# andrrizzi/tfep

Hardware: AMD Instinct MI355X
Metric: samples/s (fwd+log|detJ|) MAF+RQ-spline, 3N=3000, batch 64k (higher is better)
Workload: dtype f32

## Files before the change

include/tfep_hip.h:

```cpp
#ifndef TFEP_HIP_H
#define TFEP_HIP_H

#include <stdint.h>

#ifdef __cplusplus
extern "C" {
#endif

#define TFEP_HIP_ABI_VERSION 8

typedef enum tfep_status {
    TFEP_OK = 0,
    TFEP_ERR_INVALID_ARGUMENT = -1,
    TFEP_ERR_UNSUPPORTED = -2,
    TFEP_ERR_LAUNCH = -3
} tfep_status;

int tfep_hip_abi_version(void);
const char* tfep_last_error(void);

typedef struct tfep_param_layout {
    int64_t ld;
    int64_t stride_p;
    int64_t stride_f;
// ... 103 lines not shown

int tfep_quaternion_product(const float* x, int64_t ldx, const float* params, int64_t ldp, int inverse, float* y,
                            int64_t ldy, float* log_det_J, int accumulate, int B, int D, void* stream);

int tfep_periodic_embedding(const float* x, int64_t ldx, const int32_t* periodic_indices, int n_periodic,
                            const int32_t* nonperiodic_indices, int n_nonperiodic,
                            float lower, float upper, float* out, int64_t ldo, int B, void* stream);

int tfep_gather_columns(const float* src, int64_t lds, const int32_t* idx, int n_idx,
                        float* dst, int64_t ldd, int B, void* stream);
int tfep_scatter_columns(const float* src, int64_t lds, const int32_t* idx, int n_idx,
                         float* dst, int64_t ldd, int B, void* stream);


typedef enum tfep_fused_kind {
    TFEP_FUSED_AFFINE = 0,
    TFEP_FUSED_SPLINE = 1,
    TFEP_FUSED_SOS = 3
} tfep_fused_kind;

int tfep_fused_tile_features(void);
int tfep_fused_supported(int kind, const tfep_spline_desc* desc);
int tfep_fused_tile_columns(int kind, const tfep_spline_desc* desc);

int tfep_fused_output_transformer_forward(const float* h, int64_t ldh, const float* w, int64_t ldw,
                                          const float* bias_packed, const int32_t* k_ranges,
                                          const int32_t* tile_order,
                                          int kind, const tfep_spline_desc* desc,
                                          const float* x, int64_t ldx, float* y, int64_t ldy,
                                          const int32_t* feat_index, const int32_t* feat_tr,
                                          int n_feature_slots, double* ldj_partial,
                                          float* log_det_J, int accumulate,
                                          int B, int n_rows_w, int k_padded, void* stream);

int tfep_split_tile_k(void);
int tfep_split_rows(const float* src, int64_t ld_src, int64_t rows, int64_t cols, void* dst, int64_t ld_dst,
                    int64_t cols_padded, float* inv_scale, int per_tensor, void* stream);

int tfep_abs_reduce(const float* src, int64_t ld_src, int64_t rows, int64_t cols, int mode, float* out, void* stream);

int tfep_range_flag(const float* src, int64_t ld_src, int64_t rows, int64_t cols, int bits, int32_t* count, void* stream);
int tfep_column_absmax(const float* src, int64_t ld_src, int64_t rows, int64_t cols, float* out, void* stream);

int tfep_split_columns_scaled(const float* src, int64_t ld_src, int64_t rows, int64_t col0, int64_t cols, void* dst,
                              int64_t ld_dst, const float* inv_scale, void* stream);

int tfep_masked_weight_prepare_split(const float* weight_v, const float* weight_g, const float* mask, int out_features,
                                     int in_features, const int32_t* row_of_out, const int32_t* in_of_col, const int32_t* col_cut,
                                     void* w_split_out, int64_t ldw, int k_padded, float* inv_scale, void* stream);
int tfep_masked_weight_prepare_split_both(const float* weight_v, const float* weight_g, int out_features, int in_features,
                                          const int32_t* row_of_out, const int32_t* in_of_col, const int32_t* col_cut,
                                          void* w_split_out, int64_t ldw, float* w32_out, int64_t ldw32, int k_padded,
                                          float* inv_scale, void* stream);

int tfep_fused_output_transformer_forward_split(const void* h_split, int64_t ldh, const float* h_inv_scale,
                                                const void* w_split, int64_t ldw, const float* w_inv_scale,
                                                const float* bias_packed, const int32_t* k_ranges,
                                                const int32_t* tile_order, int kind, const tfep_spline_desc* desc,
                                                const float* x, int64_t ldx, float* y, int64_t ldy,
                                                const int32_t* feat_index, const int32_t* feat_tr, int n_feature_slots,
                                                double* ldj_partial, float* log_det_J, int accumulate, int B,
                                                int n_rows_w, int k_padded, void* stream);

int tfep_fused_saving_supported(const tfep_spline_desc* desc);
int tfep_fused_output_transformer_forward_split_saving(const void* h_split, int64_t ldh, const float* h_inv_scale,
                                                       const void* w_split, int64_t ldw, const float* w_inv_scale,
                                                       const float* bias_packed, const int32_t* k_ranges,
                                                       const int32_t* tile_order, const tfep_spline_desc* desc,
                                                       const float* x, int64_t ldx, float* y, int64_t ldy,
                                                       const int32_t* feat_index, const int32_t* feat_tr, int n_feature_slots,
                                                       double* ldj_partial, float* log_det_J, int accumulate, int B,
                                                       int n_rows_w, int k_padded, int w_feature_major, float* theta_out,
                                                       int64_t ld_theta, void* stream);

int tfep_diag_split_mfma_peak(float* scratch, int blocks, int iters, void* stream);
int tfep_diag_split_cycles(unsigned long long* out);

typedef struct tfep_inverse_block_desc {
    int32_t B, n_layers, n_steps, kind;
    float* x; int64_t ldx;
    float* xpad; int64_t ldxpad;
    const float* y; int64_t ldy;
    float* h[4]; int64_t ldh[4];
    const float* z[4]; int64_t ldz[4];
    const float* zout; int64_t ldzout;
    int32_t z_slabs[4]; int64_t z_slab_stride[4];
    int32_t zout_slabs; int64_t zout_slab_stride;
    float* log_det_J;
    const float* w[4]; int64_t ldw[4];
    const float* wout; int64_t ldwout;
    const int32_t* steps;
    const int32_t* feat_cols;
    const int32_t* feat_sel;
    const int32_t* feat_in;
    const int32_t* feat_periodic;
    const int32_t* in_cols;
    float emb_lower, emb_upper;
    int32_t cache_col0[4], cache_n_old[4];
    int32_t cache_len, max_feats;
    const tfep_spline_desc* spline;
    int32_t moebius_dim, moebius_unit_sphere;
    float moebius_max_radius;
    int32_t rows_per_wave;
    int32_t n_spline_groups;
    int32_t waves_per_workgroup;
    int32_t paired;
// ... 359 lines not shown
```

tfep_amd/_lib.py:

```python
import ctypes
import os
from ctypes import POINTER, Structure, c_char_p, c_double, c_float, c_int, c_int32, c_int64, c_void_p

import torch

_HERE = os.path.dirname(os.path.abspath(__file__))
LIB_PATH = os.environ.get('TFEP_HIP_LIB') or os.path.join(_HERE, 'lib', 'libtfep_hip.so')
ABI_VERSION = 8

_lib = None


class ParamLayout(Structure):
    _fields_ = [('ld', c_int64), ('stride_p', c_int64), ('stride_f', c_int64)]


class GemmDesc(Structure):
    _fields_ = [('x', c_void_p), ('ldx', c_int64), ('w', c_void_p), ('ldw', c_int64), ('bias', c_void_p),
                ('k_ranges', c_void_p), ('tile_order', c_void_p), ('col_map', c_void_p),
                ('y', c_void_p), ('ldy', c_int64),
                ('B', c_int32), ('N', c_int32), ('n_rows_w', c_int32), ('k_padded', c_int32),
                ('act', c_int32), ('accumulate', c_int32),
                ('elu_grad_of', c_void_p), ('ld_elu_grad_of', c_int64), ('tile_live', c_void_p),
                ('pre_add', c_void_p), ('ld_pre_add', c_int64), ('tile_n', c_int32),
# ... 39 lines not shown
                ('learn_lower_bound', c_int32), ('learn_upper_bound', c_int32),
                ('min_bin_size', c_float), ('min_slope', c_float)]


class SplineDescF64(Structure):
    _fields_ = [('x0', c_void_p), ('xf', c_void_p), ('y0', c_void_p), ('yf', c_void_p),
                ('n_bins', c_int32), ('circular', c_int32), ('identity_boundary_slopes', c_int32),
                ('learn_lower_bound', c_int32), ('learn_upper_bound', c_int32),
                ('min_bin_size', c_double), ('min_slope', c_double)]


class InverseChainF64Desc(Structure):
    _fields_ = [('B', c_int32), ('n_linears', c_int32), ('n_steps', c_int32), ('n_members', c_int32),
                ('y', c_void_p), ('ldy', c_int64), ('x', c_void_p), ('ldx', c_int64), ('log_det_J', c_void_p),
                ('a', c_void_p * 5), ('lda', c_int64 * 5), ('w', c_void_p * 5), ('ldw', c_int64 * 5), ('bias', c_void_p * 5),
                ('zout', c_void_p), ('ldzout', c_int64), ('zout_row0', c_int32), ('par_cols', c_int32), ('max_feats', c_int32),
                ('k0', c_int32 * 5), ('n_old', c_int32 * 5), ('n_cols', c_int32 * 5), ('lds_col0', c_int32 * 5),
                ('has_panel', c_int32 * 5), ('steps', c_void_p), ('feats', c_void_p), ('member_kind', c_int32 * 4),
                ('spline', SplineDescF64 * 4), ('emb_lower', c_double), ('emb_scale', c_double)]


class EgnnLayerParams(Structure):
    _fields_ = [('F', c_int32), ('G', c_int32)] + [(k, c_void_p) for k in (
        'dist_means', 'dist_log_gammas', 'msg0_w', 'msg0_b', 'msg2_w', 'msg2_b', 'att_w', 'att_b', 'ux0_w', 'ux0_b',
        'ux2_w', 'uh0_w', 'uh0_b', 'uh2_w', 'uh2_b')]


class EgnnEdgeArgs(Structure):
    _fields_ = [('B', c_int32), ('n_nodes', c_int32), ('nt', c_int32), ('split', c_int32), ('r_cutoff', c_float),
                ('speed_factor', c_float),
                ('packed', c_void_p), ('pos', c_void_p), ('dpos', c_void_p), ('P', c_void_p), ('Q', c_void_p),
                ('pq_bstride', c_int64), ('dP', c_void_p), ('dQ', c_void_p), ('pos_out', c_void_p), ('dpos_out', c_void_p),
                ('nm', c_void_p), ('dnm', c_void_p)]


class EgnnNodeArgs(Structure):
    _fields_ = [('B', c_int32), ('n_nodes', c_int32), ('nt', c_int32), ('packed', c_void_p), ('packed_next', c_void_p),
                ('h', c_void_p), ('h_bstride', c_int64), ('dh', c_void_p), ('nm', c_void_p), ('dnm', c_void_p),
                ('h_out', c_void_p), ('dh_out', c_void_p), ('P_out', c_void_p), ('Q_out', c_void_p),
                ('dP_out', c_void_p), ('dQ_out', c_void_p)]


class EgnnEdgeBwdArgs(Structure):
    _fields_ = [('B', c_int32), ('n_nodes', c_int32), ('nt', c_int32), ('split', c_int32), ('src_owned', c_int32),
                ('r_cutoff', c_float), ('speed_factor', c_float), ('packed', c_void_p), ('pos', c_void_p),
                ('P', c_void_p), ('Q', c_void_p), ('pq_bstride', c_int64), ('g_pos_out', c_void_p), ('g_nm', c_void_p),
                ('g_lane', c_void_p), ('g_pos', c_void_p)]


class EgnnNodeBwdArgs(Structure):
    _fields_ = [('B', c_int32), ('n_nodes', c_int32), ('nt', c_int32), ('packed', c_void_p), ('packed_next', c_void_p),
                ('h', c_void_p), ('h_bstride', c_int64), ('nm', c_void_p), ('g_h_next', c_void_p), ('g_P', c_void_p),
                ('g_Q', c_void_p), ('g_h', c_void_p), ('g_nm', c_void_p)]


_P = c_void_p
_SIGNATURES = {
    'tfep_hip_abi_version': (c_int, []),
    'tfep_last_error': (c_char_p, []),
    'tfep_masked_weight_prepare': (c_int, [_P, _P, _P, c_int, c_int, _P, _P, _P, c_int, _P, c_int, c_int64, _P]),
    'tfep_masked_weight_prepare_prefix': (c_int, [_P, _P, c_int, c_int, _P, _P, _P, _P, c_int, c_int64, _P]),
    'tfep_mask_k_ranges': (c_int, [_P, c_int, c_int, _P, _P, c_int, c_int, c_int, c_int, _P, _P]),
    'tfep_masked_linear_forward': (c_int, [_P, c_int64, _P, c_int64, _P, _P, _P, _P, _P, c_int64,
                                           c_int, c_int, c_int, c_int, c_int, c_int, _P]),
    'tfep_masked_linear_narrow_tile_n': (c_int, []),
    'tfep_masked_linear_tile_n': (c_int, []),
    'tfep_split_wide_tile_n': (c_int, []),
    'tfep_split_half_wide_tile_n': (c_int, []),
    'tfep_masked_linear_tile_k': (c_int, []),
    'tfep_masked_linear_tile_m': (c_int, []),
    'tfep_affine_forward': (c_int, [_P, c_int64, _P, ParamLayout, _P, c_int64, _P, c_int, c_int, c_int, _P]),
    'tfep_affine_inverse': (c_int, [_P, c_int64, _P, ParamLayout, _P, c_int64, _P, c_int, c_int, c_int, _P]),
    'tfep_sos_forward': (c_int, [_P, c_int64, _P, ParamLayout, c_int, _P, c_int64, _P, c_int, c_int, c_int, _P]),
    'tfep_sos_backward': (c_int, [_P, c_int64, _P, ParamLayout, c_int, _P, c_int64, _P, ParamLayout, _P, c_int64,
                                  c_int, c_int, _P]),
    'tfep_volume_preserving_shift': (c_int, [_P, c_int64, _P, c_int64, _P, c_float, c_float, c_int,
                                             _P, c_int64, c_int, c_int, _P]),
    'tfep_spline_n_parameters_per_feature': (c_int, [POINTER(SplineDesc)]),
    'tfep_spline_forward': (c_int, [_P, c_int64, _P, ParamLayout, POINTER(SplineDesc), _P, c_int64,
                                    _P, c_int, c_int, c_int, _P]),
    'tfep_spline_inverse': (c_int, [_P, c_int64, _P, ParamLayout, POINTER(SplineDesc), _P, c_int64,
                                    _P, c_int, c_int, c_int, _P]),
    'tfep_moebius_forward': (c_int, [_P, c_int64, _P, c_int64, c_int, c_float, c_int, c_int,
                                     _P, c_int64, _P, c_int, c_int, c_int, _P]),
    'tfep_symmetrized_moebius': (c_int, [_P, c_int64, _P, c_int64, c_int, c_double, c_int, _P, c_int64, _P, c_int, c_int,
                                         c_int, _P]),
    'tfep_symmetrized_moebius_backward': (c_int, [_P, c_int64, _P, c_int64, c_int, c_double, c_int, _P, c_int64, _P, _P,
                                                  c_int64, _P, c_int64, c_int, c_int, _P]),
    'tfep_symmetrized_moebius_f64': (c_int, [_P, c_int64, _P, c_int64, c_int, c_double, c_int, _P, c_int64, _P, c_int, c_int,
                                             c_int, _P]),
    'tfep_symmetrized_moebius_backward_f64': (c_int, [_P, c_int64, _P, c_int64, c_int, c_double, c_int, _P, c_int64, _P, _P,
                                                      c_int64, _P, c_int64, c_int, c_int, _P]),
    'tfep_quaternion_product': (c_int, [_P, c_int64, _P, c_int64, c_int, _P, c_int64, _P, c_int, c_int, c_int, _P]),
    'tfep_quaternion_product_backward': (c_int, [_P, c_int64, _P, c_int64, c_int, _P, c_int64, _P, c_int64, _P, c_int64,
                                                 c_int, c_int, _P]),
    'tfep_quaternion_product_f64': (c_int, [_P, c_int64, _P, c_int64, c_int, _P, c_int64, _P, c_int, c_int, c_int, _P]),
    'tfep_quaternion_product_backward_f64': (c_int, [_P, c_int64, _P, c_int64, c_int, _P, c_int64, _P, c_int64, _P, c_int64,
                                                     c_int, c_int, _P]),
    'tfep_moebius_forward_split_out': (c_int, [_P, c_int64, _P, c_int64, c_float, _P, c_int64, _P, c_int, _P, c_int64, _P,
                                               c_int, c_int, _P]),
    'tfep_periodic_embedding': (c_int, [_P, c_int64, _P, c_int, _P, c_int, c_float, c_float,
                                        _P, c_int64, c_int, _P]),
    'tfep_gather_columns': (c_int, [_P, c_int64, _P, c_int, _P, c_int64, c_int, _P]),
    'tfep_scatter_columns': (c_int, [_P, c_int64, _P, c_int, _P, c_int64, c_int, _P]),
    'tfep_fused_tile_features': (c_int, []),
    'tfep_fused_supported': (c_int, [c_int, POINTER(SplineDesc)]),
    'tfep_fused_tile_columns': (c_int, [c_int, POINTER(SplineDesc)]),
    'tfep_fused_output_transformer_forward': (c_int, [_P, c_int64, _P, c_int64, _P, _P, _P, c_int,
                                                      POINTER(SplineDesc), _P, c_int64, _P, c_int64,
                                                      _P, _P, c_int, _P, _P, c_int,
                                                      c_int, c_int, c_int, _P]),
    'tfep_split_tile_k': (c_int, []),
    'tfep_masked_weight_prepare_split': (c_int, [_P, _P, _P, c_int, c_int, _P, _P, _P, _P, c_int64, c_int, _P, _P]),
    'tfep_masked_weight_prepare_split_both': (c_int, [_P, _P, c_int, c_int, _P, _P, _P, _P, c_int64, _P, c_int64, c_int, _P, _P]),
    'tfep_split_rows': (c_int, [_P, c_int64, c_int64, c_int64, _P, c_int64, c_int64, _P, c_int, _P]),
    'tfep_abs_reduce': (c_int, [_P, c_int64, c_int64, c_int64, c_int, _P, _P]),
    'tfep_range_flag': (c_int, [_P, c_int64, c_int64, c_int64, c_int, _P, _P]),
    'tfep_column_absmax': (c_int, [_P, c_int64, c_int64, c_int64, _P, _P]),
    'tfep_split_columns_scaled': (c_int, [_P, c_int64, c_int64, c_int64, c_int64, _P, c_int64, _P, _P]),
    'tfep_fused_output_transformer_forward_split': (c_int, [_P, c_int64, _P, _P, c_int64, _P, _P, _P, _P, c_int,
                                                            POINTER(SplineDesc), _P, c_int64, _P, c_int64,
                                                            _P, _P, c_int, _P, _P, c_int,
                                                            c_int, c_int, c_int, _P]),
    'tfep_fused_saving_supported': (c_int, [POINTER(SplineDesc)]),
    'tfep_fused_output_transformer_forward_split_saving': (c_int, [_P, c_int64, _P, _P, c_int64, _P, _P, _P, _P,
                                                                   POINTER(SplineDesc), _P, c_int64, _P, c_int64,
                                                                   _P, _P, c_int, _P, _P, c_int,
                                                                   c_int, c_int, c_int, c_int, _P, c_int64, _P]),
    'tfep_diag_split_mfma_peak': (c_int, [_P, c_int, c_int, _P]),
    'tfep_diag_split_cycles': (c_int, [_P]),
    'tfep_inverse_block_step_ints': (c_int, []),
    'tfep_inverse_block_record_ints': (c_int, []),
    'tfep_inverse_block_lds_bytes': (c_int64, [c_int, c_int, c_int]),
    'tfep_inverse_block_lds_bytes_rows': (c_int64, [c_int, c_int, c_int, c_int]),
    'tfep_inverse_block_lds_bytes_paired': (c_int64, [c_int, c_int, c_int]),
    'tfep_inverse_block': (c_int, [POINTER(InverseBlockDesc), _P]),
    'tfep_diag_inverse_cycles': (c_int, [_P]),
    'tfep_maf_layer_tile_n': (c_int, []),
    'tfep_maf_layer_forward_split': (c_int, [POINTER(MafLayerDesc), _P]),
    'tfep_diag_maf_layer_cycles': (c_int, [_P]),
    'tfep_diag_mfma_peak': (c_int, [_P, c_int, c_int, _P]),
    'tfep_masked_linear_gemm': (c_int, [POINTER(GemmDesc), _P]),
    'tfep_transpose': (c_int, [_P, c_int64, c_int, c_int, _P, c_int64, _P]),
    'tfep_transpose_split': (c_int, [_P, c_int64, c_int, c_int, _P, c_int64, c_int, c_int, _P, _P, _P]),
    'tfep_transpose_split_rows': (c_int, [_P, c_int64, c_int, c_int, _P, c_int64, _P]),
    'tfep_column_sums_absmax': (c_int, [_P, c_int64, c_int, c_int, _P, c_int, _P, _P]),
    'tfep_column_sums': (c_int, [_P, c_int64, c_int, c_int, _P, c_int, _P]),
    'tfep_add_inplace': (c_int, [_P, c_int64, _P, c_int64, c_int, c_int, _P]),
    'tfep_affine_backward': (c_int, [_P, c_int64, _P, ParamLayout, _P, c_int64, _P, _P, ParamLayout, _P, c_int64,
                                     c_int, c_int, _P]),
    'tfep_spline_backward': (c_int, [_P, c_int64, _P, ParamLayout, POINTER(SplineDesc), _P, c_int64, _P, _P,
                                     ParamLayout, _P, c_int64, c_int, c_int, _P]),
    'tfep_moebius_backward': (c_int, [_P, c_int64, _P, c_int64, c_int, c_float, c_int, c_int, _P, c_int64, _P,
                                      _P, c_int64, _P, c_int64, c_int, c_int, _P]),
    'tfep_copy_2d': (c_int, [_P, c_int64, _P, c_int64, c_int, c_int, _P]),
    'tfep_weight_norm_backward': (c_int, [_P, c_int64, _P, _P, _P, c_int, c_int, _P, _P, _P, _P, _P]),
    'tfep_weight_norm_backward_prefix': (c_int, [_P, c_int64, _P, _P, c_int, c_int, _P, _P, _P, _P, _P, _P]),
    'tfep_periodic_embedding_backward': (c_int, [_P, c_int64, _P, c_int, _P, c_int, c_float, c_float, _P, c_int64,
                                                 _P, c_int64, c_int, _P]),
    'tfep_tfep_reduce': (c_int, [_P, _P, _P, _P, _P, c_float, c_int, c_int, _P, _P, _P]),
    'tfep_tfep_reduce_workspace_doubles': (c_int, [c_int]),
    'tfep_bootstrap_fep': (c_int, [_P, _P, _P, _P, c_int64, c_int64, c_int64, c_float, _P, _P]),
    'tfep_egnn_tile': (c_int, [c_int, c_int]),
    'tfep_egnn_packed_floats': (c_int64, [c_int]),
    'tfep_egnn_pack_layer': (c_int, [POINTER(EgnnLayerParams), c_int, _P, _P]),
    'tfep_egnn_embed': (c_int, [_P, c_int, c_int, c_float, _P, _P, c_int, _P, _P, POINTER(EgnnLayerParams), c_int,
# ... 138 lines not shown
```

tfep_amd/build.py:

```python
import fcntl
import os
import subprocess
import sys

HERE = os.path.dirname(os.path.abspath(__file__))
CSRC = os.path.join(HERE, 'csrc')
LIB_DIR = os.path.join(HERE, 'lib')
LIB_PATH = os.path.join(LIB_DIR, 'libtfep_hip.so')
SOURCES = ['transformers.hip', 'masked_linear.hip', 'split_gemm.hip', 'split_gemm_layouts.hip', 'inverse_block.hip',
           'reduce.hip', 'backward.hip', 'egnn.hip', 'maf_layer.hip', 'masked_linear_f64.hip',
           'spline_f64.hip', 'inverse_block_f64.hip', 'flipembed.hip']
EXTRA_FLAGS = {'egnn.hip': ['-fno-slp-vectorize']}


def _hipcc():
    for cand in (os.environ.get('HIPCC'), '/opt/rocm/bin/hipcc', 'hipcc'):
        if cand and (os.path.isabs(cand) and os.path.exists(cand) or not os.path.isabs(cand)):
            return cand
    raise RuntimeError('hipcc not found')


def _headers():
    deps = [os.path.join(CSRC, f) for f in os.listdir(CSRC) if f.endswith('.h')]
    deps.append(os.path.join(os.path.dirname(HERE), 'include', 'tfep_hip.h'))
    return deps


def needs_build():
    if not os.path.exists(LIB_PATH):
        return True
    t = os.path.getmtime(LIB_PATH)
    deps = [os.path.join(CSRC, f) for f in SOURCES] + _headers()
    return any(os.path.getmtime(d) > t for d in deps)


def build_probe(out_path, extra_flags, verbose=True):
    import tempfile
    tmp = tempfile.mkdtemp(prefix='tfep_probe_')
    objs, procs = [], []
    for src in SOURCES:
        obj = os.path.join(tmp, src.replace('.hip', '.o'))
        objs.append(obj)
        cmd = [_hipcc(), '-O3', '-std=c++17', '--offload-arch=gfx950', '-fPIC', '-fno-gpu-rdc', '-Wno-unused-result',
               *EXTRA_FLAGS.get(src, []), *extra_flags, '-c', os.path.join(CSRC, src), '-o', obj]
        if verbose:
            print(' '.join(cmd), flush=True)
        procs.append((src, subprocess.Popen(cmd)))
    for src, p in procs:
        if p.wait() != 0:
            raise RuntimeError(f'hipcc failed on {src}')
    subprocess.check_call([_hipcc(), '--offload-arch=gfx950', '-shared', '-fPIC', '-o', out_path] + objs)
    return out_path


def build(force=False, verbose=True):
    if not force and not needs_build():
        return LIB_PATH
    os.makedirs(LIB_DIR, exist_ok=True)
    with open(os.path.join(LIB_DIR, '.build.lock'), 'w') as lock:
        fcntl.flock(lock, fcntl.LOCK_EX)
        try:
            if not force and not needs_build():
                return LIB_PATH
            return _build_locked(force, verbose)
# ... 46 lines not shown
```

tfep_amd/nn/conditioners/made.py:

```python
from typing import Literal, Optional, Sequence, Union

import os

import numpy as np

import torch

from ... import ops
from ...utils.misc import ensure_tensor_sequence
from .. import masked
from .conditioner import Conditioner



def _round_robin(x, length, err_msg=None):
    n_rounds, n_rem = divmod(length, len(x))
    if n_rounds == 0:
        if err_msg is None:
            err_msg = f'Length {length} is smaller than the array (len={len(x)}).'
        raise ValueError(err_msg)
    out = x.repeat(n_rounds)
    if n_rem != 0:
        out = torch.cat([out, x[:n_rem]])
    return out
# ... 414 lines not shown
            old = plan.get('packed_fingerprint')
            stale = old is None or not torch.equal(old, fingerprint)
        plan['packed_checked'] = fingerprint
        if stale:
            for k in [k for k in plan if isinstance(k, tuple) and k[0] in ('packed', 'packed_split')]:
                del plan[k]
            plan['packed_versions'] = versions
        plan['packed_fingerprint'] = fingerprint
        return True

    def begin_call(self):
        self.__dict__['_fp_memo'] = None

    def _param_fingerprint(self):
        parts = []
        for lin in self._linears():
            for t in lin.parameters():
                flat = t.detach().reshape(-1)
                parts.append(flat[::1021].sum(dtype=torch.float64))
                parts.append(flat[:64].sum(dtype=torch.float64))
        return torch.stack(parts) if parts else torch.zeros(0)

    def _mask_prefix_cuts(self, plan, li, lin):
        if os.environ.get('TFEP_MASK_PREFIX', '1') == '0':
            return None
        key = ('col_cut', li)
        cached = plan.get(key)
        version = lin.mask._version
        if cached is not None and cached[0] == version:
            return cached[1]
        if torch.cuda.is_current_stream_capturing():
            return None
        in_of_col = plan['in_of_col'][li]
        gather = None if in_of_col is None else in_of_col.long()
        cuts, prefix = [], True
        with torch.no_grad():
            for r0 in range(0, lin.mask.shape[0], 4096):
                m = lin.mask[r0:r0 + 4096]
                m = m if gather is None else m[:, gather]
                if not bool((((m == 0) | (m == 1)).all() & (m[:, 1:] <= m[:, :-1]).all()).item()):
                    prefix = False
                    break
                cuts.append(m.sum(dim=1).to(torch.int32))
        cut = torch.cat(cuts).contiguous() if prefix and cuts else None
        plan[key] = (version, cut)
        return cut

    def prepack_split_async(self, device, stream, last=None):
        plan = self.plan(device)
        lins = self._linears()
        self._packed_ahead = None
        if self.cache_packed_weights and not self._frozen or self.dtype == torch.float64:
            return
        stream.wait_stream(torch.cuda.current_stream(device))
        items = {}
        with torch.cuda.stream(stream):
            for li, lin in enumerate(lins):
                if li == len(lins) - 1 and last is not None:
                    items[(li, last[1])] = self._pack_layer_split(plan, li, lin, row_of_out=last[0], n_rows=last[1])
                else:
                    items[(li, plan['n_pad'][li])] = self._pack_layer_split(plan, li, lin)
            event = stream.record_event()
        self._packed_ahead = dict(items=items, event=event, joined=False, device=device, versions=self._param_versions())

    def _param_versions(self):
        return tuple((t._version, t.data_ptr()) for lin in self._linears() for t in (*lin.parameters(), lin.mask))

    def drop_packed_ahead(self):
        self._packed_ahead = None

    def _embed(self, x):
        return x

    def frozen_weights(self):
        return _FrozenWeights(self)

    def forward_hidden(self, x, split=False):
        ops.check_device_tensor(x, 'x', self.dtype)
        x = self._embed(x)
        if x.shape[1] != self.dimension_in:
            raise ValueError(f'expected {self.dimension_in} input features, got {x.shape[1]}')
        plan = self.plan(x.device)
        lins = self._linears()
        if self.dtype == torch.float64:
            split = False
        h = ops.pad_columns(x, plan['k_pad'][0], self.dtype)
        for li, lin in enumerate(lins[:-1]):
            if split:
                ws, w_inv, b, _ = self._pack_layer_split(plan, li, lin)
                hs, h_inv = ops.split_rows(h, plan['k_pad'][li])
                h = ops.masked_linear_split(hs, h_inv, ws, w_inv, b, plan['n_pad'][li], k_ranges=plan['k_ranges'][li],
                                            act=1, tile_order=plan['tile_order'][li])
            else:
                w, b = self._pack_layer(plan, li, lin)
                h = ops.masked_linear_packed(h, w, b, plan['n_pad'][li], k_ranges=plan['k_ranges'][li], act=1,
                                             tile_order=plan['tile_order'][li])
        return h, plan

    def split_worthwhile(self, batch=None):
        n = self.__dict__.get('_n_weights')
        if n is None:
            n = self.__dict__['_n_weights'] = sum(lin.mask.numel() for lin in self._linears())
        by_batch = self.split_by_batch and batch is not None and n * int(batch) >= (1 << 35)
        return n >= (1 << 22) or by_batch

    def forward_hidden_split(self, x, split_hint=None):
        ops.check_device_tensor(x, 'x')
        if split_hint is None:
            split_hint = getattr(x, '_tfep_split', None)
        hint_version = x._version
        x_in = x
        x = self._embed(x)
        if x is not x_in:
            split_hint = None
        if x.shape[1] != self.dimension_in:
            raise ValueError(f'expected {self.dimension_in} input features, got {x.shape[1]}')
# ... 70 lines not shown
```

tfep_amd/nn/flows/autoregressive.py:

```python
import ctypes
import math
import os
from typing import Optional, Sequence

import torch

from ... import _lib, ops
from ...utils.misc import ensure_tensor_sequence
from ..conditioners.made import MADE
from ..embeddings.mafembed import FlipInvariantEmbedding, MixedEmbedding, PeriodicEmbedding
from ..transformers.affine import AffineTransformer, VolumePreservingShiftTransformer
from ..transformers.mixed import MixedTransformer, check_float64_members
from ..transformers.moebius import MoebiusTransformer, SymmetrizedMoebiusTransformer
from ..transformers.quatprod import QuaternionProductTransformer
from ..transformers.sos import SOSPolynomialTransformer
from ..transformers.spline import NeuralSplineTransformer
from .sequential import _side_stream

_FUSED_AFFINE, _FUSED_SPLINE, _FUSED_MIXED, _FUSED_SOS = 0, 1, 2, 3


class AutoregressiveFlow(torch.nn.Module):

    def __init__(
# ... 178 lines not shown
            members = [(self._member_fused_kind(t), t, ind.cpu().long(), off)
                       for t, ind, off in zip(tr._transformers, tr._indices, tr.host_splits()) if len(ind) > 0]
        else:
            members = [(kind, tr, None, 0)]
        i32 = dict(device=device, dtype=torch.int32)
        li = len(mplan['n_pad']) - 1
        row_of_out = torch.full((last.out_features,), -1, dtype=torch.long, device='cpu')
        groups, base = [], 0
        for k_g, t_g, rel, off in members:
            n_g = n_tr if rel is None else len(rel)
            P = 2 if k_g == _FUSED_AFFINE else t_g.n_parameters_per_feature
            P_real = 1 if self._is_plain_shift(t_g) else P
            if off + P_real * n_g > last.out_features:
                raise ValueError('conditioner output does not match the transformer parameters')
            desc = t_g.config(device).desc if k_g == _FUSED_SPLINE else (
                ops.sos_fused_desc(t_g.n_polynomials) if k_g == _FUSED_SOS else None)
            tile_cols = lib.tfep_fused_tile_columns(k_g, ctypes.byref(desc) if desc is not None else None)
            FT = tile_cols // (16 * P)
            n_slots = ops.round_up(n_g, 16 * FT)
            deg = made._degrees[-1][off:off + n_g].cpu()
            order = torch.argsort(deg, stable=True)
            slot_of = torch.empty_like(order)
            slot_of[order] = torch.arange(n_g, device='cpu')
            feat_tr = torch.zeros(n_slots, dtype=torch.long, device='cpu')
            feat_tr[:n_g] = order
            feat_index = torch.full((n_slots,), -1, dtype=torch.long, device='cpu')
            feat_index[:n_g] = (cols_tr if rel is None else cols_tr[rel])[order]
            sl = slot_of.repeat(P_real)
            pp = torch.arange(P_real, device='cpu').repeat_interleave(n_g)
            local = (sl // (16 * FT)) * tile_cols + (((sl // 16) % FT) * P + pp) * 16 + (sl % 16)
            n_tiles = n_slots // (16 * FT)
            row_of_out[off:off + P_real * n_g] = base + local
            grp = {'kind': k_g, 'transformer': t_g, 'P': P, 'FT': FT, 'n_slots': n_slots, 'n_rows': n_tiles * tile_cols,
                   'base': base, 'feat_index': feat_index.to(**i32), 'feat_tr': feat_tr.to(**i32)}
            grp['k_ranges'] = ops.mask_k_ranges(last.mask[off:off + P_real * n_g], tile_cols, n_tiles, mplan['k_pad'][li],
                                                local.to(**i32), mplan['col_of_in'][li])
            grp['tile_order'] = ops.heavy_first_order(grp['k_ranges'])
            groups.append(grp)
            base += grp['n_rows']
        if bool((row_of_out < 0).any()):
            raise ValueError('conditioner output does not match the transformer parameters')
        fp = {'kind': kind, 'groups': groups, 'n_rows': base, 'row_of_out': row_of_out.to(**i32), 'li': li}
        self._dev[key] = fp
        return fp

    def _forward_fused(self, x, kind):
        x, ldx = _lib.rows(x, 'x')
        B, D = x.shape
        tables = self._tables(x.device)
        fp = self._fused_plan(x.device, kind, tables)
        made = self._conditioner
        split = self._use_split_gemm(B)
        if split:
            h, h_inv, mplan = made.forward_hidden_split(x)
            w, w_inv, b, _ = made._pack_layer_split(mplan, fp['li'], made.layers[-1], row_of_out=fp['row_of_out'],
                                                    n_rows=fp['n_rows'])
        else:
            h, mplan = made.forward_hidden(x)
            w, b = made._pack_layer(mplan, fp['li'], made.layers[-1], row_of_out=fp['row_of_out'], n_rows=fp['n_rows'])
        prof = getattr(self, '_profile_events', None)
        if prof is not None:
            ev0, ev1 = torch.cuda.Event(enable_timing=True), torch.cuda.Event(enable_timing=True)
            ev0.record(torch.cuda.current_stream(x.device))
        y = x.clone() if self.has_fixed_indices else torch.empty(x.shape, dtype=x.dtype, device=x.device)
        ldj = None
        for grp in fp['groups']:
            if grp['kind'] == _FUSED_SPLINE:
                cfg, hst = grp['transformer'].config(x.device), grp['transformer'].host()
                spl = (cfg.x0, cfg.xf, cfg.y0, cfg.yf, hst['n_bins'], hst['circular'], hst['identity'], hst['learn_lower'],
                       hst['learn_upper'], hst['min_bin'], hst['min_slope'])
            elif grp['kind'] == _FUSED_SOS:
                spl = (None, None, None, None, grp['transformer'].n_polynomials, False, False, False, False, 0.0, 0.0)
            else:
                spl = (None, None, None, None, 0, False, False, False, False, 0.0, 0.0)
            r0, r1 = grp['base'], grp['base'] + grp['n_rows']
            l = torch.ops.tfep.fused_output_transformer_(
                h, h_inv if split else None, w[r0:r1], w_inv if split else None, b[r0:r1], grp['k_ranges'],
                grp['tile_order'], grp['kind'], x, y, grp['feat_index'], grp['feat_tr'], grp['n_slots'], grp['n_rows'], *spl)
            ldj = l if ldj is None else ldj + l
        if prof is not None:
            ev1.record(torch.cuda.current_stream(x.device))
            prof.append((ev0, ev1))
        if split:
            made.drop_packed_ahead()
        return y, ldj

    layer_kernel = None

    def _layer_kernel_ok(self, x):
        want = self.layer_kernel if self.layer_kernel is not None else os.environ.get('TFEP_LAYER_KERNEL', '0') == '1'
        if not want or self.fused is False:
            return False
        made, tr = self._conditioner, self._transformer
        if type(tr) is not MoebiusTransformer or tr.dimension != 2 or not isinstance(made, MADE):
            return False
        if getattr(made, 'embedding', None) is not None or self.has_fixed_indices or len(self._conditioner_indices) > 0:
            return False
        lins = made._linears()
        if not (2 <= len(lins) <= 4) or max(l.out_features for l in lins) > 4096 or lins[-1].out_features != x.shape[1]:
            return False
        if x.shape[1] % 2 or made.dimension_in != x.shape[1]:
            return False
        return True

    def _layer_plan(self, device):
        made = self._conditioner
# ... 1446 lines not shown
```

tfep_amd/ops.py:

```python
import ctypes
import os

import torch

from . import _lib
from ._lib import ParamLayout, SplineDesc, SplineDescF64, call, check_device_tensor, ptr, rows, stream_of


def _dtype(x):
    return torch.float64 if isinstance(x, torch.Tensor) and x.dtype == torch.float64 else torch.float32


def _sfx(dtype):
    return '_f64' if dtype == torch.float64 else ''


def _ldj_out(log_det_J, B, like, dtype=torch.float32):
    if log_det_J is None:
        return torch.empty(B, dtype=dtype, device=like.device), 0
    check_device_tensor(log_det_J, 'log_det_J', dtype)
    if log_det_J.shape != (B,) or not log_det_J.is_contiguous():
        raise ValueError('log_det_J must be a contiguous (batch,) tensor')
    return log_det_J, 1

# ... 558 lines not shown
def range_flag(tensors, bits=19):
    tensors = [t for t in tensors if t is not None and t.numel() > 0]
    if not tensors:
        return 0
    count = torch.zeros(1, dtype=torch.int32, device=tensors[0].device)
    for t in tensors:
        check_device_tensor(t, 'range_flag input')
        if t.dim() != 2 or t.stride(1) != 1:
            t = t.reshape(t.shape[0], -1).contiguous() if t.dim() > 1 else t.reshape(1, -1).contiguous()
        call('tfep_range_flag', ptr(t), t.stride(0) if t.shape[0] > 1 else t.shape[1], t.shape[0], t.shape[1], int(bits),
             ptr(count), stream_of(t))
    return int(count.item())


def range_flag_device(tensors, bits=19, count=None):
    tensors = [t for t in tensors if t is not None and t.numel() > 0]
    if not tensors:
        return count
    if count is None:
        count = zeros(1, dtype=torch.int32, device=tensors[0].device)
    for t in tensors:
        check_device_tensor(t, 'range_flag input')
        if t.dim() != 2 or t.stride(1) != 1:
            t = t.reshape(t.shape[0], -1).contiguous() if t.dim() > 1 else t.reshape(1, -1).contiguous()
        call('tfep_range_flag', ptr(t), t.stride(0) if t.shape[0] > 1 else t.shape[1], t.shape[0], t.shape[1], int(bits),
             ptr(count), stream_of(t))
    return count


def abs_reduce(x, what):
    x, ldx = rows(x, 'x')
    mode = {'row_max': 0, 'max_row_sum': 1}[what]
    out = torch.empty(x.shape[0] if mode == 0 else 1, dtype=torch.float32, device=x.device)
    call('tfep_abs_reduce', ptr(x), ldx, x.shape[0], x.shape[1], mode, ptr(out), stream_of(x))
    return out


def pow2_inv_scale(bound):
    e = torch.floor(torch.log2(bound.clamp_min(1e-30).double()))
    return torch.exp2(e - 14.0).float()


def masked_weight_prepare_split(weight_v, weight_g, mask, row_of_out, in_of_col, out, inv_scale, col_cut=None):
    check_device_tensor(weight_v, 'weight')
    if inv_scale.numel() < 4:
        raise ValueError('inv_scale must have 4 entries')
    N, K = weight_v.shape
    v_c = weight_v.contiguous()
    g_c = None if weight_g is None else weight_g.contiguous()
    m_c = None if mask is None else mask.contiguous()
    call('tfep_masked_weight_prepare_split', ptr(v_c), ptr(g_c), ptr(m_c), N, K, ptr(row_of_out), ptr(in_of_col), ptr(col_cut),
         ptr(out), out.shape[1], out.shape[1], ptr(inv_scale), stream_of(weight_v))
    return out, inv_scale


def masked_linear_split(x_split, x_inv_scale, w_split, w_inv_scale, bias, n_out, k_ranges=None, act=0, out=None,
                        tile_order=None, split_out=False, bias_absmax=None, k_split=1):
    B = x_split.shape[0]
    n_rows_w, k_padded = w_split.shape
    if out is None:
        out = torch.empty((B, n_out) if k_split <= 1 else (k_split, B, n_out), dtype=torch.float32, device=x_split.device)
    d = _lib.GemmDesc()
    if split_out:
        if bias_absmax is None:
            bias_absmax = abs_reduce(bias.reshape(1, -1), 'row_max') if bias is not None else zeros(1, device=out.device)
        y_inv = torch.empty(max(B, 1), dtype=torch.float32, device=out.device)
        d.split_out, d.y_inv_scale = 1, y_inv.data_ptr()
        d.w_l1max, d.bias_absmax = w_inv_scale.data_ptr() + 8, bias_absmax.data_ptr()
    d.x, d.ldx = x_split.data_ptr(), x_split.shape[1]
    d.w, d.ldw = w_split.data_ptr(), k_padded
    d.bias = bias.data_ptr() if bias is not None else None
    d.k_ranges = k_ranges.data_ptr() if k_ranges is not None else None
    d.tile_order = tile_order.data_ptr() if tile_order is not None else None
    d.col_map = None
    d.y, d.ldy = out.data_ptr(), out.shape[-1]
    d.B, d.N, d.n_rows_w, d.k_padded, d.act, d.accumulate = B, n_out, n_rows_w, k_padded, int(act), 0
    d.split, d.x_inv_scale, d.w_inv_scale = 1, x_inv_scale.data_ptr(), w_inv_scale.data_ptr()
    if k_split > 1:
        d.k_split, d.slab_stride = int(k_split), out.shape[-2] * out.shape[-1]
    call('tfep_masked_linear_gemm', ctypes.byref(d), stream_of(x_split))
    return (out, y_inv) if split_out else out



def tfep_reduce(target_potentials, log_det_J=None, ref_potentials=None, log_weights=None, bias=None,
                kT=1.0, ignore_nan=False):
    dt = _dtype(target_potentials)
    t = check_device_tensor(target_potentials.contiguous(), 'target_potentials', dt)
    N = t.numel()
    opt = []
    for v, n in ((log_det_J, 'log_det_J'), (ref_potentials, 'ref_potentials'), (log_weights, 'log_weights'),
                 (bias, 'bias')):
        if v is not None:
            v = check_device_tensor(v.contiguous(), n, dt)
            if v.numel() != N:
                raise ValueError(f'{n} must have {N} elements')
        opt.append(v)
    nws = _lib.load().tfep_tfep_reduce_workspace_doubles(N)
    ws = torch.empty(nws, dtype=torch.float64, device=t.device)
    out = torch.empty(9, dtype=torch.float64, device=t.device)
    call('tfep_tfep_reduce' + _sfx(dt), ptr(t), ptr(opt[0]), ptr(opt[1]), ptr(opt[2]), ptr(opt[3]), float(kT),
         int(bool(ignore_nan)), N, ptr(ws), ptr(out), stream_of(t))
    return out
```

Measured before the change: 80140.

## Pack all MADE layer weights in one persistent multi-matrix kernel

Adds a new HIP kernel that packs every weight-normed, prefix-masked MADE linear layer into the split fp16 hi/lo format in a single persistent launch. Rows are distributed across a CU-sized grid and the next row is prefetched into registers while the current one is written. A small kernel computes the per-matrix gain max first. The flow forward now triggers this pack eagerly on the current stream, replacing several per-layer pack launches. The cost is a more complex kernel and new constraints on row width and matrix count.

```diff
diff --git a/include/tfep_hip.h b/include/tfep_hip.h
--- a/include/tfep_hip.h
+++ b/include/tfep_hip.h
@@ -179,6 +179,21 @@
                                           const int32_t* row_of_out, const int32_t* in_of_col, const int32_t* col_cut,
                                           void* w_split_out, int64_t ldw, float* w32_out, int64_t ldw32, int k_padded,
                                           float* inv_scale, void* stream);
+
+#define TFEP_PACK_MAX_MATRICES 4
+typedef struct {
+    const float* weight_v;
+    const float* weight_g;
+    const int32_t* row_of_out;
+    const int32_t* in_of_col;
+    const int32_t* col_cut;
+    void* w_split_out;
+    float* inv_scale;
+    int64_t ldw;
+    int32_t out_features, in_features, k_padded, n_rows_padded;
+    int32_t zero_suffix, reserved;
+} tfep_pack_matrix_desc;
+int tfep_masked_weight_prepare_split_layer(const tfep_pack_matrix_desc* matrices, int n_matrices, void* stream);
 
 int tfep_fused_output_transformer_forward_split(const void* h_split, int64_t ldh, const float* h_inv_scale,
                                                 const void* w_split, int64_t ldw, const float* w_inv_scale,
diff --git a/tfep_amd/_lib.py b/tfep_amd/_lib.py
--- a/tfep_amd/_lib.py
+++ b/tfep_amd/_lib.py
@@ -115,6 +115,13 @@
     _fields_ = [('B', c_int32), ('n_nodes', c_int32), ('nt', c_int32), ('packed', c_void_p), ('packed_next', c_void_p),
                 ('h', c_void_p), ('h_bstride', c_int64), ('nm', c_void_p), ('g_h_next', c_void_p), ('g_P', c_void_p),
                 ('g_Q', c_void_p), ('g_h', c_void_p), ('g_nm', c_void_p)]
+
+
+class PackMatrixDesc(Structure):
+    _fields_ = [('weight_v', c_void_p), ('weight_g', c_void_p), ('row_of_out', c_void_p), ('in_of_col', c_void_p),
+                ('col_cut', c_void_p), ('w_split_out', c_void_p), ('inv_scale', c_void_p), ('ldw', c_int64),
+                ('out_features', c_int32), ('in_features', c_int32), ('k_padded', c_int32), ('n_rows_padded', c_int32),
+                ('zero_suffix', c_int32), ('reserved', c_int32)]
 
 
 _P = c_void_p
@@ -175,6 +182,7 @@
                                                       c_int, c_int, c_int, _P]),
     'tfep_split_tile_k': (c_int, []),
     'tfep_masked_weight_prepare_split': (c_int, [_P, _P, _P, c_int, c_int, _P, _P, _P, _P, c_int64, c_int, _P, _P]),
+    'tfep_masked_weight_prepare_split_layer': (c_int, [_P, c_int, _P]),
     'tfep_masked_weight_prepare_split_both': (c_int, [_P, _P, c_int, c_int, _P, _P, _P, _P, c_int64, _P, c_int64, c_int, _P, _P]),
     'tfep_split_rows': (c_int, [_P, c_int64, c_int64, c_int64, _P, c_int64, c_int64, _P, c_int, _P]),
     'tfep_abs_reduce': (c_int, [_P, c_int64, c_int64, c_int64, c_int, _P, _P]),
diff --git a/tfep_amd/build.py b/tfep_amd/build.py
--- a/tfep_amd/build.py
+++ b/tfep_amd/build.py
@@ -9,7 +9,7 @@
 LIB_PATH = os.path.join(LIB_DIR, 'libtfep_hip.so')
 SOURCES = ['transformers.hip', 'masked_linear.hip', 'split_gemm.hip', 'split_gemm_layouts.hip', 'inverse_block.hip',
            'reduce.hip', 'backward.hip', 'egnn.hip', 'maf_layer.hip', 'masked_linear_f64.hip',
-           'spline_f64.hip', 'inverse_block_f64.hip', 'flipembed.hip']
+           'spline_f64.hip', 'inverse_block_f64.hip', 'flipembed.hip', 'weight_pack.hip']
 EXTRA_FLAGS = {'egnn.hip': ['-fno-slp-vectorize']}
 
 
diff --git a/tfep_amd/csrc/weight_pack.hip b/tfep_amd/csrc/weight_pack.hip
--- /dev/null
+++ b/tfep_amd/csrc/weight_pack.hip
@@ -0,0 +1,270 @@
+#include <stdlib.h>
+
+#include "common.h"
+#include "gemm_common.h"
+#include "split_gemm_kernel.h"
+
+namespace tfep {
+
+constexpr int PL_THREADS = 512;
+constexpr int PL_MAX = TFEP_PACK_MAX_MATRICES;
+struct PackMatrix {
+    const float* v; const float* g;
+    const int32_t* row_of_out; const int32_t* in_of_col; const int32_t* col_cut;
+    uint4* w_out; float* inv_scale;
+    int64_t ldw;
+    int32_t N, K, k_padded, row0, zero_suffix, wave_l1;
+};
+struct PackLayerArgs {
+    PackMatrix m[PL_MAX];
+    int32_t n, total_rows;
+};
+
+__global__ void __launch_bounds__(256) pack_layer_scale_kernel(PackLayerArgs a) {
+    __shared__ float part[4];
+    const PackMatrix& d = a.m[blockIdx.x];
+    float m = 0.f;
+    if (d.g)
+        for (int i = threadIdx.x; i < d.N; i += 256) m = fmaxf(m, fabsf(d.g[i]));
+#pragma unroll
+    for (int off = 32; off > 0; off >>= 1) m = fmaxf(m, __shfl_xor(m, off, 64));
+    if ((threadIdx.x & 63) == 0) part[threadIdx.x >> 6] = m;
+    __syncthreads();
+    if (threadIdx.x == 0) {
+        uint32_t* bits = reinterpret_cast<uint32_t*>(d.inv_scale);
+        bits[1] = __float_as_uint(fmaxf(fmaxf(part[0], part[1]), fmaxf(part[2], part[3])));
+        bits[2] = 0u;
+    }
+}
+
+__global__ void __launch_bounds__(PL_THREADS, 4) weight_prepare_split_layer_kernel(PackLayerArgs a) {
+    extern __shared__ float4 pl_smem4[];
+    float* const smem = reinterpret_cast<float*>(pl_smem4);
+    __shared__ float s_wn;
+    const int tid = threadIdx.x, lane = tid & 63, wave = tid >> 6;
+    const int stride = gridDim.x;
+
+    auto matrix_of = [&](int r) {
+        int m = 0;
+#pragma unroll
+        for (int i = 1; i < PL_MAX; ++i)
+            if (i < a.n && r >= a.m[i].row0) m = i;
+        return m;
+    };
+    auto cut_of = [&](int r) {
+        if (r >= a.total_rows) return 0;
+        const PackMatrix& d = a.m[matrix_of(r)];
+        return min(d.col_cut[r - d.row0], d.K);
+    };
+
+    float4 q[8];
+    float q_head = 0.f, q_tail = 0.f;
+    auto fetch = [&](int r) {
+#pragma unroll
+        for (int u = 0; u < 8; ++u) q[u] = make_float4(0.f, 0.f, 0.f, 0.f);
+        if (r >= a.total_rows) return;
+        const PackMatrix& d = a.m[matrix_of(r)];
+        const int K = d.K;
+        const float* vr = d.v + (int64_t)(r - d.row0) * K;
+        const int head = min(K, (int)(((16u - (uint32_t)((uintptr_t)vr & 15u)) & 15u) >> 2));
+        const int n4 = (K - head) >> 2;
+        const float4* v4 = reinterpret_cast<const float4*>(vr + head);
+#pragma unroll
+        for (int u = 0; u < 8; ++u) {
+            const int i = tid + u * PL_THREADS;
+            if (i < n4) q[u] = v4[i];
+        }
+        if (tid < head) q_head = vr[tid];
+        if (head + 4 * n4 + tid < K) q_tail = vr[head + 4 * n4 + tid];
+    };
+
+    int r = blockIdx.x;
+    if (r >= a.total_rows) return;
+    int cut = cut_of(r), cut_next = cut_of(r + stride);
+    fetch(r);
+    for (; r < a.total_rows; r += stride) {
+        const PackMatrix& d = a.m[matrix_of(r)];
+        const int o = r - d.row0, K = d.K;
+        const float* vr = d.v + (int64_t)o * K;
+        const int head = min(K, (int)(((16u - (uint32_t)((uintptr_t)vr & 15u)) & 15u) >> 2));
+        const int n4 = (K - head) >> 2;
+        const int pad = (4 - head) & 3;
+        float* const srow = smem + pad;
+        const int n_groups = (cut + 7) >> 3;
+        const bool vec_idx = d.in_of_col && ((uintptr_t)d.in_of_col & 15u) == 0;
+        int4 ia[4], ib[4];
+#pragma unroll
+        for (int u = 0; u < 4; ++u) {
+            const int g8 = tid + u * PL_THREADS;
+            ia[u] = ib[u] = make_int4(0, 0, 0, 0);
+            if (vec_idx && g8 < n_groups && g8 * 8 + 8 <= K) {
+                ia[u] = reinterpret_cast<const int4*>(d.in_of_col)[2 * g8];
+                ib[u] = reinterpret_cast<const int4*>(d.in_of_col)[2 * g8 + 1];
+            }
+        }
+        {
+            float4* s4 = reinterpret_cast<float4*>(srow + head);
+#pragma unroll
+            for (int u = 0; u < 8; ++u) {
+                const int i = tid + u * PL_THREADS;
+                if (i < n4) s4[i] = q[u];
+            }
+            if (tid < head) srow[tid] = q_head;
+            if (head + 4 * n4 + tid < K) srow[head + 4 * n4 + tid] = q_tail;
+        }
+        const float gain = d.g ? d.g[o] : 0.f;
+        const float s = pow2_scale_for(__uint_as_float(*reinterpret_cast<const uint32_t*>(d.inv_scale + 1)));
+        __syncthreads();
+        float e[4][8];
+#pragma unroll
+        for (int u = 0; u < 4; ++u) {
+            const int g8 = tid + u * PL_THREADS;
+            int idx[8];
+            if (vec_idx && g8 * 8 + 8 <= K) {
+                const int4 x = ia[u], y = ib[u];
+                idx[0] = x.x; idx[1] = x.y; idx[2] = x.z; idx[3] = x.w; idx[4] = y.x; idx[5] = y.y; idx[6] = y.z; idx[7] = y.w;
+            } else {
+#pragma unroll
+                for (int j = 0; j < 8; ++j) {
+                    const int c = g8 * 8 + j;
+                    idx[j] = (d.in_of_col && c < cut) ? d.in_of_col[c] : c;
+                }
+            }
+#pragma unroll
+            for (int j = 0; j < 8; ++j) {
+                const int c = g8 * 8 + j;
+                e[u][j] = c < cut ? srow[min((unsigned)idx[j], (unsigned)(K - 1))] : 0.f;
+            }
+        }
+        const int cut_now = cut;
+        const int r_next = r + stride;
+        fetch(r_next);
+        cut = cut_next;
+        cut_next = cut_of(r_next + stride);
+        if (wave == PL_THREADS / 64 - 1) {
+            float wn = 1.0f;
+            if (d.g) {
+                float ss = 0.f;
+                for (int i = lane; i < K; i += 64) ss += srow[i] * srow[i];
+                ss = wave_sum(ss);
+                wn = gain / sqrtf(ss);
+            }
+            if (lane == 0) s_wn = wn;
+            if (d.wave_l1) {
+                float l1 = 0.f;
+                for (int g8 = lane; g8 < n_groups; g8 += 64) {
+#pragma unroll
+                    for (int j = 0; j < 8; ++j) {
+                        const int c = g8 * 8 + j;
+                        float val = 0.f;
+                        if (c < cut_now) val = srow[min((unsigned)(d.in_of_col ? d.in_of_col[c] : c), (unsigned)(K - 1))] * wn;
+                        l1 += fabsf(val);
+                    }
+                }
+                l1 = wave_sum(l1);
+                if (lane == 0 && l1 < INFINITY) {
+                    uint32_t* mx = reinterpret_cast<uint32_t*>(d.inv_scale + 2);
+                    if (__float_as_uint(l1) > __atomic_load_n(mx, __ATOMIC_RELAXED)) atomicMax(mx, __float_as_uint(l1));
+                }
+            }
+        }
+        __syncthreads();
+        const float wn = s_wn;
+        if (o == 0 && tid == 0) d.inv_scale[0] = 1.0f / s;
+        const int64_t orow = d.row_of_out ? d.row_of_out[o] : o;
+        uint4* dr = d.w_out + orow * (d.ldw / 4);
+        float l1 = 0.f;
+#pragma unroll
+        for (int u = 0; u < 4; ++u) {
+            const int g8 = tid + u * PL_THREADS;
+            if (g8 >= n_groups) break;
+            f16x8 hi, lo;
+#pragma unroll
+            for (int j = 0; j < 8; ++j) {
+                const int c = g8 * 8 + j;
+                float val = 0.f;
+                if (c < cut_now) val = e[u][j] * wn;
+                l1 += fabsf(val);
+                val *= s;
+                const _Float16 h = (_Float16)val;
+                hi[j] = h;
+                lo[j] = (_Float16)(val - (float)h);
+            }
+            dr[g8 * 2] = *reinterpret_cast<uint4*>(&hi);
+            dr[g8 * 2 + 1] = *reinterpret_cast<uint4*>(&lo);
+        }
+        if (d.zero_suffix) {
+            const uint4 z = make_uint4(0u, 0u, 0u, 0u);
+            for (int g8 = n_groups + tid; g8 * 8 < d.k_padded; g8 += PL_THREADS) dr[g8 * 2] = dr[g8 * 2 + 1] = z;
+        }
+        if (!d.wave_l1) {
+            l1 = wave_sum(l1);
+            if (lane == 0 && l1 < INFINITY) {
+                uint32_t* mx = reinterpret_cast<uint32_t*>(d.inv_scale + 2);
+                if (__float_as_uint(l1) > __atomic_load_n(mx, __ATOMIC_RELAXED)) atomicMax(mx, __float_as_uint(l1));
+            }
+        }
+    }
+}
+
+}
+
+using namespace tfep;
+
+extern "C" {
+
+int tfep_masked_weight_prepare_split_layer(const tfep_pack_matrix_desc* matrices, int n_matrices, void* stream) {
+    TFEP_REQUIRE(matrices && n_matrices >= 1 && n_matrices <= PL_MAX, "masked_weight_prepare_split_layer: 1 .. %d matrices", PL_MAX);
+    hipStream_t s = (hipStream_t)stream;
+    int order[PL_MAX];
+    for (int i = 0; i < n_matrices; ++i) {
+        int j = i;
+        for (; j > 0 && matrices[order[j - 1]].in_features < matrices[i].in_features; --j) order[j] = order[j - 1];
+        order[j] = i;
+    }
+    PackLayerArgs a = {};
+    int64_t total = 0;
+    int max_k = 0;
+    for (int i = 0; i < n_matrices; ++i) {
+        const tfep_pack_matrix_desc& m = matrices[order[i]];
+        TFEP_REQUIRE(m.weight_v && m.weight_g && m.col_cut && m.w_split_out && m.inv_scale, "masked_weight_prepare_split_layer: NULL pointer (matrix %d)", order[i]);
+        TFEP_REQUIRE(m.out_features >= 1 && m.in_features >= 1, "masked_weight_prepare_split_layer: empty matrix %d", order[i]);
+        TFEP_REQUIRE((size_t)m.in_features * 4 + 16 <= 64 * 1024, "masked_weight_prepare_split_layer: rows of at most 16380 weights (matrix %d has %d)",
+                     order[i], m.in_features);
+        TFEP_REQUIRE(m.k_padded >= m.in_features && m.k_padded % SBK == 0 && m.ldw >= m.k_padded && m.ldw % 4 == 0,
+                     "masked_weight_prepare_split_layer: k_padded=%d must be a multiple of %d >= in_features, ldw >= k_padded (matrix %d)",
+                     m.k_padded, SBK, order[i]);
+        TFEP_REQUIRE(m.n_rows_padded >= m.out_features, "masked_weight_prepare_split_layer: n_rows_padded < out_features (matrix %d)", order[i]);
+        TFEP_REQUIRE((uintptr_t)m.w_split_out % 16 == 0 && (uintptr_t)m.weight_v % 4 == 0 && (uintptr_t)m.inv_scale % 4 == 0,
+                     "masked_weight_prepare_split_layer: misaligned pointer (matrix %d)", order[i]);
+        TFEP_REQUIRE((!m.weight_g || (uintptr_t)m.weight_g % 4 == 0) && (!m.row_of_out || (uintptr_t)m.row_of_out % 4 == 0) &&
+                     (!m.in_of_col || (uintptr_t)m.in_of_col % 4 == 0) && (uintptr_t)m.col_cut % 4 == 0,
+                     "masked_weight_prepare_split_layer: misaligned pointer (matrix %d)", order[i]);
+        PackMatrix& d = a.m[i];
+        d.v = m.weight_v; d.g = m.weight_g; d.row_of_out = m.row_of_out; d.in_of_col = m.in_of_col; d.col_cut = m.col_cut;
+        d.w_out = (uint4*)m.w_split_out; d.inv_scale = m.inv_scale; d.ldw = m.ldw;
+        d.N = m.out_features; d.K = m.in_features; d.k_padded = m.k_padded; d.row0 = (int32_t)total;
+        d.zero_suffix = m.zero_suffix != 0;
+        d.wave_l1 = !(m.in_features >= 8192 && (size_t)m.in_features * 4 <= 64 * 1024);
+        total += m.out_features;
+        max_k = m.in_features > max_k ? m.in_features : max_k;
+    }
+    TFEP_REQUIRE(total <= 0x7fffffffLL / 2, "masked_weight_prepare_split_layer: too many rows");
+    a.n = n_matrices;
+    a.total_rows = (int32_t)total;
+    pack_layer_scale_kernel<<<(unsigned)n_matrices, 256, 0, s>>>(a);
+    static int n_cus[TFEP_MAX_DEVICES] = {};
+    int& cus = n_cus[current_device_slot()];
+    if (cus == 0) {
+        int dev = 0, v = 0;
+        if (hipGetDevice(&dev) != hipSuccess || hipDeviceGetAttribute(&v, hipDeviceAttributeMultiprocessorCount, dev) != hipSuccess || v <= 0) v = 256;
+        cus = v;
+    }
+    static const int per_cu = env_int("TFEP_PACK_WGS_PER_CU", 2);
+    const int64_t want = (int64_t)cus * (per_cu > 0 ? per_cu : 2);
+    const unsigned grid = (unsigned)(total < want ? total : want);
+    weight_prepare_split_layer_kernel<<<grid, PL_THREADS, (size_t)max_k * 4 + 16, s>>>(a);
+    return check_launch("weight_prepare_split_layer_kernel");
+}
+
+}
diff --git a/tfep_amd/nn/conditioners/made.py b/tfep_amd/nn/conditioners/made.py
--- a/tfep_amd/nn/conditioners/made.py
+++ b/tfep_amd/nn/conditioners/made.py
@@ -490,16 +490,65 @@
         self._packed_ahead = None
         if self.cache_packed_weights and not self._frozen or self.dtype == torch.float64:
             return
+        if stream is None:
+            if self._keep_packed(plan):
+                return
+            items = self._pack_all_split(plan, lins, last)
+            if items is not None:
+                self._packed_ahead = dict(items=items, event=None, joined=True, device=device, versions=self._param_versions())
+            return
         stream.wait_stream(torch.cuda.current_stream(device))
-        items = {}
         with torch.cuda.stream(stream):
-            for li, lin in enumerate(lins):
-                if li == len(lins) - 1 and last is not None:
-                    items[(li, last[1])] = self._pack_layer_split(plan, li, lin, row_of_out=last[0], n_rows=last[1])
-                else:
-                    items[(li, plan['n_pad'][li])] = self._pack_layer_split(plan, li, lin)
+            items = self._pack_all_split(plan, lins, last)
+            if items is None:
+                items = {}
+                for li, lin in enumerate(lins):
+                    if li == len(lins) - 1 and last is not None:
+                        items[(li, last[1])] = self._pack_layer_split(plan, li, lin, row_of_out=last[0], n_rows=last[1])
+                    else:
+                        items[(li, plan['n_pad'][li])] = self._pack_layer_split(plan, li, lin)
             event = stream.record_event()
         self._packed_ahead = dict(items=items, event=event, joined=False, device=device, versions=self._param_versions())
+
+    def pack_split_now(self, device, last=None):
+        ahead = self._packed_ahead
+        if ahead is None or ahead['versions'] != self._param_versions():
+            self.prepack_split_async(device, None, last=last)
+
+    def _pack_all_split(self, plan, lins, last=None):
+        if os.environ.get('TFEP_PACK_LAYER', '1') == '0' or not 1 <= len(lins) <= ops.PACK_LAYER_MAX_MATRICES:
+            return None
+        if not all(lin.has_weight_norm and lin.mask.shape[1] <= ops.PACK_LAYER_MAX_COLUMNS for lin in lins):
+            return None
+        cuts = [self._mask_prefix_cuts(plan, li, lin) for li, lin in enumerate(lins)]
+        if all(c is None for c in cuts):
+            return None
+        todo, bufs, items = [], [], {}
+        for li, lin in enumerate(lins):
+            row_of_out, n_rows = plan['row_of_out'][li], plan['n_pad'][li]
+            if li == len(lins) - 1 and last is not None:
+                row_of_out, n_rows = last
+            if cuts[li] is None:
+                items[(li, n_rows)] = self._pack_layer_split(plan, li, lin, row_of_out=row_of_out, n_rows=n_rows)
+                continue
+            v = lin.weight_v.detach()
+            key = ('ws', li, n_rows, None if row_of_out is None else row_of_out.data_ptr())
+            buf = plan.get(key)
+            if buf is None:
+                buf = (ops.zeros(n_rows, plan['k_pad'][li], dtype=torch.float32, device=v.device),
+                       ops.zeros(4, dtype=torch.float32, device=v.device), row_of_out)
+                plan[key] = buf
+            mask_key, mask_now = ('ws_mask',) + key[1:], (lin.mask._version, cuts[li].data_ptr())
+            todo.append(dict(weight_v=v, weight_g=lin.weight_g.detach(), row_of_out=row_of_out, in_of_col=plan['in_of_col'][li],
+                             col_cut=cuts[li], out=buf[0], inv_scale=buf[1], zero_suffix=plan.get(mask_key) != mask_now))
+            plan[mask_key] = mask_now
+            bufs.append((li, n_rows, row_of_out, buf))
+        ops.masked_weight_prepare_split_layer(todo)
+        for li, n_rows, row_of_out, buf in bufs:
+            lin = lins[li]
+            bias = self._pack_bias(lin, row_of_out, n_rows)
+            items[(li, n_rows)] = (buf[0], buf[1], bias, ops.abs_reduce(bias.reshape(1, -1), 'row_max'))
+        return items
 
     def _param_versions(self):
         return tuple((t._version, t.data_ptr()) for lin in self._linears() for t in (*lin.parameters(), lin.mask))
diff --git a/tfep_amd/nn/flows/autoregressive.py b/tfep_amd/nn/flows/autoregressive.py
--- a/tfep_amd/nn/flows/autoregressive.py
+++ b/tfep_amd/nn/flows/autoregressive.py
@@ -254,6 +254,7 @@
         made = self._conditioner
         split = self._use_split_gemm(B)
         if split:
+            made.pack_split_now(x.device, last=(fp['row_of_out'], fp['n_rows']))
             h, h_inv, mplan = made.forward_hidden_split(x)
             w, w_inv, b, _ = made._pack_layer_split(mplan, fp['li'], made.layers[-1], row_of_out=fp['row_of_out'],
                                                     n_rows=fp['n_rows'])
diff --git a/tfep_amd/ops.py b/tfep_amd/ops.py
--- a/tfep_amd/ops.py
+++ b/tfep_amd/ops.py
@@ -634,6 +634,30 @@
     call('tfep_masked_weight_prepare_split', ptr(v_c), ptr(g_c), ptr(m_c), N, K, ptr(row_of_out), ptr(in_of_col), ptr(col_cut),
          ptr(out), out.shape[1], out.shape[1], ptr(inv_scale), stream_of(weight_v))
     return out, inv_scale
+
+
+PACK_LAYER_MAX_COLUMNS = 16380
+PACK_LAYER_MAX_MATRICES = 4
+
+
+def masked_weight_prepare_split_layer(items):
+    descs = (_lib.PackMatrixDesc * len(items))()
+    keep = []
+    for d, it in zip(descs, items):
+        v, out, inv = it['weight_v'], it['out'], it['inv_scale']
+        check_device_tensor(v, 'weight')
+        if inv.numel() < 4:
+            raise ValueError('inv_scale must have 4 entries')
+        if it['weight_g'] is None or it['col_cut'] is None:
+            raise ValueError('masked_weight_prepare_split_layer takes weight-normed matrices with prefix masks only')
+        v_c, g_c = v.contiguous(), it['weight_g'].contiguous()
+        keep += [v_c, g_c]
+        d.weight_v, d.weight_g = ptr(v_c), ptr(g_c)
+        d.row_of_out, d.in_of_col, d.col_cut = ptr(it.get('row_of_out')), ptr(it.get('in_of_col')), ptr(it['col_cut'])
+        d.w_split_out, d.inv_scale, d.ldw = ptr(out), ptr(inv), out.shape[1]
+        d.out_features, d.in_features, d.k_padded, d.n_rows_padded = v.shape[0], v.shape[1], out.shape[1], out.shape[0]
+        d.zero_suffix = 1 if it.get('zero_suffix') else 0
+    call('tfep_masked_weight_prepare_split_layer', ctypes.cast(descs, ctypes.c_void_p), len(items), stream_of(items[0]['weight_v']))
 
 
 def masked_linear_split(x_split, x_inv_scale, w_split, w_inv_scale, bias, n_out, k_ranges=None, act=0, out=None,
```

Result: no change. 80070, median of 2 (-0.1%).
